# CrystalAnalyst/Lsm

Hardware: AMD Instinct MI355X
Metric: GiB/s device-resident SSTable block encode+decode, 4 KiB blocks, 1/2/4/8 GPU (higher is better)
Workload: dtype u8; 1 GPU; U: 1048576 blocks/GPU x block_size 4096, decode + re-encode (16-B uniform keys, 100-B values); blocks_per_gpu=1048576, entries_per_gpu=32474205, encoded_bytes_per_gpu=4226189427, decoded_bytes_per_gpu=4286595060, block_size=4096, segments_per_gpu=2045, parallelism=block-sharded x1 (no data-path collective), encode_output=segments packed (lsmblk_encode_batch), rccl_world=1

## Files before the change

### lsm_amd/csrc/lsmblk_dev.hpp

```cpp
#pragma once

#include <hip/hip_runtime.h>
#include <hip/hip_ext.h>

#include <cstdint>
#include <cstdlib>
#include <cstring>
#include <mutex>
#include <new>
#include <type_traits>
#include <vector>

#include "lsmblk.h"
#include "lsmblk_keys.hpp"

namespace {

constexpr uint32_t kSpinLimit = 1u << 22;

constexpr bool kDiag = LSMBLK_DIAG_BUILD != 0;
__device__ __forceinline__ uint32_t diag_mask(uint32_t skip) { return kDiag ? skip : 0u; }

__device__ __forceinline__ uint32_t lane_id() { return threadIdx.x & 63u; }
__device__ __forceinline__ uint32_t uni(uint32_t x) { return __builtin_amdgcn_readfirstlane(x); }
// ... 695 lines not shown
      cap = bytes = 0;
    }
    const hipError_t e = status ? hipExtMallocWithFlags(&mem, nb, kStatusFlags) : hipMallocAsync(&mem, nb, st);
    if (e != hipSuccess) {
      mem = nullptr;
      return LSMBLK_E_NOMEM;
    }
    if (fresh) *fresh = true;
    if (hipMemsetAsync(mem, 0, nb, st) != hipSuccess) return LSMBLK_E_HIP;
    cap = nc;
    bytes = nb;
    return LSMBLK_OK;
  }
  bool zero(hipStream_t st) const { return !bytes || hipMemsetAsync(mem, 0, bytes, st) == hipSuccess; }
  void release() {
    if (!mem) return;
    if (status) (void)hipFree(mem);
    else (void)hipFreeAsync(mem, nullptr);
    mem = nullptr;
    cap = bytes = 0;
  }
};
template <typename T>
struct DevBuf : DevBufBase {
  using DevBufBase::DevBufBase;
  T* get() const { return static_cast<T*>(mem); }
  operator T*() const { return get(); }
  int grow(hipStream_t st, uint64_t need, uint64_t per, bool* fresh = nullptr) {
    return grow_bytes(st, need, per * sizeof(T), fresh);
  }
};

struct lsmblk_ctx {
  int device = 0;
  std::mutex mu;
  DevBufBase* bufs = nullptr;
  uint32_t* counters = nullptr;
  DevBuf<uint32_t> dec_agg{bufs, false};
  void* crc_tabs = nullptr;
  DevBuf<uint64_t> tile_sum{bufs, false};
  DevBuf<uint64_t> tile_pre{bufs, false};
  DevBuf<uint64_t> seg_agg{bufs, true};
  DevBuf<uint64_t> seg_inc{bufs, true};
  DevBuf<uint32_t> rec_first{bufs, false};
  DevBuf<uint32_t> blk_first{bufs, false};
  DevBuf<uint32_t> ent{bufs, false};
  DevBuf<uint32_t> big_list{bufs, false};
  DevBuf<uint32_t> blk_sz{bufs, false};
  DevBuf<uint64_t> frec{bufs, true};
  DevBuf<uint64_t> fdone{bufs, true};
  DevBuf<uint32_t> fwnb{bufs, false};
  DevBuf<uint8_t> fbig{bufs, false};
  bool fuse_on = false;
  bool plan_pipe = false;
  uint32_t emit_mode = 0;
  uint32_t emit_grid = 0;
  DevBuf<uint64_t> lag_gran{bufs, true};
  uint64_t lag_blk_cap = 0;
  uint32_t rot_poison = 0;
  uint32_t emit_poison = 0;
  bool dec_two_pass = false;
  uint32_t dec_lag = kDecLagDefault;
  uint64_t dec_lag_bytes = kDecLagBytesDefault;
  uint64_t* dbg = nullptr;
  bool dbg_on = false;
  uint32_t epoch = 0;
  uint32_t poll = 0;
  uint32_t skip = 0;
  bool timing = false;
  struct KLog {
    const char* name;
    int slot;
    hipEvent_t e0, e1;
  };
  std::vector<KLog> klog;
  uint64_t klog_n = 0;
  uint64_t klog_total = 0;
  uint64_t dec_log0 = 0, dec_log1 = 0, enc_log0 = 0, enc_log1 = 0;
  DevBuf<uint32_t> meta_rec{bufs, false};
  DevBuf<uint64_t> meta_pos{bufs, false};
  DevBuf<uint64_t> meta_tile{bufs, false};
  DevBuf<uint32_t> meta_crc{bufs, false};
  uint64_t* meta_cstats = nullptr;
  DevBuf<uint32_t> filt_keep{bufs, false};
  DevBuf<uint64_t> filt_tile{bufs, false};
  DevBuf<uint8_t> cws{bufs, false};
  DevBuf<uint32_t> vcrc{bufs, false};
  hipStream_t aux = nullptr;
  hipEvent_t fork_ev = nullptr, join_ev = nullptr;
  DevBuf<uint8_t> sws{bufs, false};
  uint32_t scan_units = kScanUnitsDefault;
  DevBuf<uint8_t> rws{bufs, false};
  uint64_t shard_n = 0, shard_m = 0, shard_target = 0;
  uint32_t shard_block_size = 0, shard_flags = 0, shard_sst_cap = 0;
  bool shard_ready = false;
};

inline thread_local lsmblk_ctx* tl_launch_ctx = nullptr;
constexpr uint32_t kKLogCap = 16384;

namespace {
struct DeviceGuard {
  int prev = -1;
  bool ok = false;
  lsmblk_ctx* prev_ctx = nullptr;
  explicit DeviceGuard(int dev, lsmblk_ctx* c = nullptr) {
    if (hipGetDevice(&prev) != hipSuccess) prev = -1;
// ... 135 lines not shown
```

### lsm_amd/csrc/lsmblk_gpu.hip

```cpp
#include "lsmblk_dev.hpp"

namespace {


struct DecodeArgs {
  const uint8_t* blocks;
  const uint64_t* blk_off;
  uint64_t nblk;
  uint8_t* keys;
  uint32_t* key_off;
  uint8_t* vals;
  uint32_t* val_off;
  uint64_t* ts;
  uint64_t entry_cap, key_cap, val_cap;
  uint64_t* stats;
  const uint32_t* agg;
  const uint64_t* tile_pre;
  uint32_t tail;
  uint64_t* blk_ent;
  uint32_t skip;
  uint64_t* bagg;
  uint64_t* bbase;
  uint64_t* tagg;
  uint64_t* tinc;
// ... 1182 lines not shown
#pragma unroll
            for (uint32_t d = 0; d < 4; ++d) t[d] = uint32_t(__builtin_ctzg(P[d] ^ Q[d], 32)) >> 3;
            const uint32_t z16 = t[0] < 4 ? t[0] : t[1] < 4 ? 4 + t[1] : t[2] < 4 ? 8 + t[2] : 12 + t[3];
            const uint32_t zd = z16 >> 2;
            if (z16 < m) {
              lcp = z16;
              w0 = zd == 0 ? P[0] : zd == 1 ? P[1] : zd == 2 ? P[2] : P[3];
              w1 = zd == 0 ? Q[0] : zd == 1 ? Q[1] : zd == 2 ? Q[2] : Q[3];
            }
            done = z16 < m || m <= 16;
            if (!done) {
              for (uint32_t d = 4; 4 * d < m; ++d) {
                const uint32_t y0 = K.dw(pp[i] + 4 * d), y1 = K.dw(kp[i] + 4 * d);
                if (y0 != y1) {
                  const uint32_t z = 4 * d + (__builtin_ctz(y0 ^ y1) >> 3);
                  if (z < m) {
                    lcp = z;
                    w0 = y0;
                    w1 = y1;
                  }
                  break;
                }
              }
            }
          } else {
            const KeyDiff kd = key_diff(K, pp[i], pl, kp[i], kl);
            lcp = kd.lcp, w0 = kd.w0, w1 = kd.w1;
          }
          const uint32_t sh = 8 * (lcp & 3);
          const bool sorted = lcp == m ? pl <= kl : ((w0 >> sh) & 0xFF) < ((w1 >> sh) & 0xFF);
          al = (lcp < kAlcpLcp ? lcp : kAlcpLcp) | (sorted ? 0u : kAlcpUnsorted);
        }
        CR[x] = inv ? kl : kl + (v1[i] - v0[i]);
        CA[x] = al;
      }
    }
    __builtin_amdgcn_fence(__ATOMIC_RELEASE, "workgroup");
    if (l == 0) __hip_atomic_store(prod, cend - s0, __ATOMIC_RELAXED, __HIP_MEMORY_SCOPE_WORKGROUP);
  }
  if (tr && l == 0) {
    tr[5] = __builtin_amdgcn_s_memrealtime();
    tr[6] = waited;
  }
}

struct WalkRing {
  const uint32_t* CR;
  const uint32_t* CA;
  uint32_t* cons;
  const uint32_t* prod;
  uint32_t S0;
  uint32_t known = 0;
  bool stalled = false;
};

template <class Sink>
__device__ __forceinline__ void walk_segment(const PlanArgs& a, const ArenaKeys& K, WalkRing& R, uint32_t s0, uint32_t s1,
                                             uint32_t& err, uint32_t& nb, uint64_t& bytes, Sink&& sink, uint64_t* tr,
                                             uint64_t& waited, uint64_t& windows) {
  const uint32_t l = lane_id();
  auto need = [&](uint32_t j0, uint32_t wend) {
    __hip_atomic_store(R.cons, j0 - R.S0, __ATOMIC_RELAXED, __HIP_MEMORY_SCOPE_WORKGROUP);
    if (tr) ++windows;
    if (wend - R.S0 > R.known && !R.stalled) {
      const uint64_t w0 = tr ? __builtin_amdgcn_s_memrealtime() : 0;
      uint32_t spins = 0;
      while ((R.known = __hip_atomic_load(R.prod, __ATOMIC_RELAXED, __HIP_MEMORY_SCOPE_WORKGROUP)) < wend - R.S0) {
        if (++spins > kSpinMax) {
          err |= LSMBLK_ERR_TIMEOUT;
          R.stalled = true;
          break;
        }
        __builtin_amdgcn_s_sleep(1);
      }
      if (tr) waited += __builtin_amdgcn_s_memrealtime() - w0;
      __builtin_amdgcn_fence(__ATOMIC_ACQUIRE, "workgroup");
    }
  };
  const uint32_t* const CR = R.CR;
  const uint32_t* const CA = R.CA;
  const uint32_t S0 = R.S0;
  nb = 0;
  bytes = 0;
  const uint64_t bs = a.block_size;
  const bool narrow = bs < (1ull << 30);
  for (uint32_t s = s0; s < s1;) {
    uint64_t carry = 2;
    uint32_t pmin = kAlcpLcp;
    bool direct = false;
    uint32_t sp = 0, sl = 0;
    uint32_t j0 = s;
    const uint32_t aend = s1 - s < 64 ? s1 : s + 64;
    need(s, aend);
    if (!(diag_mask(a.skip) & (1u << 17))) {
      const bool valid = s + l < s1;
      uint32_t r = 0, al = kAlcpLcp;
      if (valid) {
        const uint32_t x = (s + l - S0) & (kRing - 1);
        r = CR[x];
        if (l) al = CA[x];
      }
      if (narrow && __ballot((al & kAlcpUnsorted) || (valid && r >= (1u << 25) - 16)) == 0) {
        const uint32_t mn = wave_incl_min31(al);
        const uint32_t g32 = valid ? r + 16 - (l ? mn : 0u) : 0u;
        const uint32_t i32 = wave_incl_scan32(g32);
        const uint32_t b32 = 2 + i32 - g32;
        const uint64_t m = __ballot(l && (!valid || b32 + r + 14 > uint32_t(bs)));
        if (m) {
          const uint32_t f = uint32_t(__builtin_ctzll(m));
          const uint32_t size = uint32_t(__builtin_amdgcn_readlane(b32, f));
          sink(s, s + f, size, nb, bytes);
          ++nb;
          bytes += size;
          s += f;
          continue;
// ... 179 lines not shown
      if (kl == 0) err |= LSMBLK_ERR_EMPTY_KEY;
      uint32_t al = 0;
      if (e != s0) {
        const uint32_t pl = kp - pp, m = pl < kl ? pl : kl;
        uint32_t lcp = m, w0 = 0, w1 = 0;
        if (K.lead + kp + 16 <= klim && K.lead + pp + 16 <= klim) {
          const uint32_t Pw[4] = {xp[i].x, xp[i].y, xp[i].z, xp[i].w}, Qw[4] = {xk[i].x, xk[i].y, xk[i].z, xk[i].w};
          uint32_t t[4];
#pragma unroll
          for (uint32_t d = 0; d < 4; ++d) t[d] = uint32_t(__builtin_ctzg(Pw[d] ^ Qw[d], 32)) >> 3;
          const uint32_t z16 = t[0] < 4 ? t[0] : t[1] < 4 ? 4 + t[1] : t[2] < 4 ? 8 + t[2] : 12 + t[3];
          const uint32_t zd = z16 >> 2;
          if (z16 < m) {
            lcp = z16;
            w0 = zd == 0 ? Pw[0] : zd == 1 ? Pw[1] : zd == 2 ? Pw[2] : Pw[3];
            w1 = zd == 0 ? Qw[0] : zd == 1 ? Qw[1] : zd == 2 ? Qw[2] : Qw[3];
          }
          if (!(z16 < m || m <= 16)) {
            for (uint32_t d = 4; 4 * d < m; ++d) {
              const uint32_t y0 = K.dw(pp + 4 * d), y1 = K.dw(kp + 4 * d);
              if (y0 != y1) {
                const uint32_t z = 4 * d + (__builtin_ctz(y0 ^ y1) >> 3);
                if (z < m) {
                  lcp = z;
                  w0 = y0;
                  w1 = y1;
                }
                break;
              }
            }
          }
        } else {
          const KeyDiff kd = key_diff(K, pp, pl, kp, kl);
          lcp = kd.lcp, w0 = kd.w0, w1 = kd.w1;
        }
        const uint32_t sh = 8 * (lcp & 3);
        const bool sorted = lcp == m ? pl <= kl : ((w0 >> sh) & 0xFF) < ((w1 >> sh) & 0xFF);
        al = (lcp < kAlcpLcp ? lcp : kAlcpLcp) | (sorted ? 0u : kAlcpUnsorted);
      }
      CR[x] = inv ? kl : kl + (P.v1[i] - P.v0[i]);
      CA[x] = al;
    }
    __builtin_amdgcn_fence(__ATOMIC_RELEASE, "workgroup");
    if (l == 0) __hip_atomic_store(prod, cend - s0, __ATOMIC_RELAXED, __HIP_MEMORY_SCOPE_WORKGROUP);
    prod_offs_land(Pn);
    P = Pn;
  }
  if (tr && l == 0) {
    tr[5] = __builtin_amdgcn_s_memrealtime();
    tr[6] = waited;
  }
}

__global__ __launch_bounds__(kWalkThreads) __attribute__((amdgpu_waves_per_eu(4))) void plan_walk_kernel(PlanArgs a0) {
  const PlanArgs a = resolve(a0);
  static_assert(kRing >= 2 * kChunk && (kRing & (kRing - 1)) == 0, "plan ring size");
  __shared__ uint32_t crec[4][kRing], calcp[4][kRing];
  const uint32_t l = lane_id();
  __shared__ uint32_t hand_g[4], hand_prod[4], hand_cons[4];
  const uint32_t wv = wave_id(), ww = wv & 3;
  if (wv < 4) {
    const uint32_t t = take_ticket(a.ticket);
    if (l == 0) {
      hand_g[wv] = t;
      hand_prod[wv] = 0;
      hand_cons[wv] = 0;
    }
  }
  __syncthreads();
  const uint32_t g = uni(hand_g[ww]);
  uint32_t* CR = crec[ww];
  uint32_t* CA = calcp[ww];
  if (g >= a.nseg) return;
  uint32_t err = 0;
  uint32_t s0 = uni(a.seg_start[g]), s1 = uni(a.seg_start[g + 1]);
  if ((!a.span && g == 0 && s0 != 0) || (!a.span && g == a.nseg - 1 && uint64_t(s1) != a.n) || s0 > s1 ||
      uint64_t(s1) > a.n) {
    err |= LSMBLK_ERR_SEGMENTS;
    s1 = s0 = (s0 > a.n ? uint32_t(a.n) : s0);
    if (s1 < s0) s1 = s0;
  }
  const ArenaKeys K = plan_keys(a);
  uint64_t* const tr = kDiag && a.dbg && g < kDbgTiles ? a.dbg + 16 + 8 * uint64_t(g) : nullptr;
  if (wv >= 4) {
    if (a.pipe_helper) plan_produce_pipe(a, K, s0, s1, CR, CA, &hand_prod[ww], &hand_cons[ww], err, tr);
    else plan_produce(a, K, s0, s1, CR, CA, &hand_prod[ww], &hand_cons[ww], err, tr);
    const uint32_t werr = (__ballot(err & LSMBLK_ERR_EMPTY_KEY) ? LSMBLK_ERR_EMPTY_KEY : 0u) |
                          (__ballot(err & LSMBLK_ERR_MALFORMED) ? LSMBLK_ERR_MALFORMED : 0u) |
                          (__ballot(err & LSMBLK_ERR_TIMEOUT) ? LSMBLK_ERR_TIMEOUT : 0u);
    raise_err(a.stats, werr);
    return;
  }
  uint64_t waited = 0, windows = 0;
  if (tr && l == 0) tr[0] = __builtin_amdgcn_s_memrealtime();
  WalkRing R{CR, CA, &hand_cons[ww], &hand_prod[ww], s0};
  uint32_t nb = 0;
  uint64_t bytes = 0;
  walk_segment(a, K, R, s0, s1, err, nb, bytes,
               [&](uint32_t first, uint32_t, uint32_t size, uint32_t i, uint64_t) {
                 if (l == 0) {
                   a.rec_first[s0 + i] = first;
                   a.sz[s0 + i] = size;
                 }
               },
               tr, waited, windows);
  if (tr && l == 0) {
    tr[1] = __builtin_amdgcn_s_memrealtime();
    tr[2] = waited;
    tr[3] = windows;
    tr[7] = nb | (uint64_t(__builtin_amdgcn_s_getreg(0xF804)) << 32) | (uint64_t(__builtin_amdgcn_s_getreg(0x1814) & 0xF) << 56);
  }
  bytes += uint64_t(a.frame) * nb;
  __builtin_amdgcn_fence(__ATOMIC_RELEASE, "agent");
  asm volatile("s_waitcnt vmcnt(0)" ::: "memory");
  __builtin_amdgcn_fence(__ATOMIC_ACQUIRE, "agent");
  uint64_t agg[2] = {nb, bytes};
  uint64_t excl[2] = {0, 0};
  if (g == 0) {
    publish<2>(a.inc, g, agg, a.tag, 2, a.poll);
  } else {
    publish<2>(a.agg, g, agg, a.tag, 1, a.poll);
    if (!lookback<2>(a.agg, a.inc, g, a.tag, a.poll, excl)) err |= LSMBLK_ERR_TIMEOUT;
    const uint64_t inc[2] = {excl[0] + agg[0], excl[1] + agg[1]};
    publish<2>(a.inc, g, inc, a.tag, 2, a.poll);
  }
  uint64_t O0 = excl[1];
  if (a.seg_out) O0 = (err & LSMBLK_ERR_SEGMENTS) ? 0ull : seg_slot(a.key_off, a.val_off, 0u, s0, a.frame);
  const uint64_t B0 = excl[0];
  if (a.seg_out && l == 0) {
    a.seg_out[2ull * g] = O0;
    a.seg_out[2ull * g + 1] = bytes;
  }
  uint64_t oc = O0;
  for (uint32_t c = 0; c < nb; c += 64) {
    const uint32_t i = c + l;
    uint32_t sz = 0, first = 0;
    if (i < nb) {
      first = a.rec_first[s0 + i];
      sz = a.sz[s0 + i];
    }
    const uint64_t ext = i < nb ? uint64_t(sz) + a.frame : 0ull;
    const uint64_t incl = wave_incl_scan<uint64_t>(ext);
    if (i < nb) {
      const uint64_t bi = B0 + i;
      a.blk_first[bi] = first;
      if (a.blk_sz) a.blk_sz[bi] = sz;
      if (bi < a.blk_cap) a.blk_off[bi] = oc + incl - ext;
    }
    oc += __shfl(incl, 63, 64);
  }
  if (g == a.nseg - 1 && l == 0) {
    const uint64_t Bt = B0 + nb, Ot = O0 + bytes;
    a.blk_first[Bt] = a.span ? s1 : uint32_t(a.n);
    if (Bt < a.blk_cap) a.blk_off[Bt] = Ot;
    a.stats[0] = Bt;
    a.stats[1] = excl[1] + bytes;
    if (Bt + 1 > a.blk_cap || Ot > a.out_cap) err |= LSMBLK_ERR_CAPACITY;
  }
// ... 648 lines not shown
    y = ny;
    fp = nfp;
    fl = nfl;
  }
  raise_err(a.stats, err);
}

__global__ __launch_bounds__(256) void emit_poison_kernel(uint32_t* blk_first, const uint64_t* stats) {
  if (stats[3] & kPlanFatal) return;
  const uint64_t nblk = stats[0], b = 1 + 5 * (uint64_t(blockIdx.x) * 256 + threadIdx.x);
  if (b < nblk) blk_first[b] = blk_first[b + 1] + 1;
}

struct FuseArgs {
  PlanArgs p;
  EmitArgs e;
  uint64_t* rec;
  uint64_t* wdone;
  uint32_t* wnb;
  uint64_t* seg_out;
  uint8_t* bigr;
  uint32_t nwalk;
  uint32_t spw;
  uint32_t walk_wgs;
  uint32_t per_walker;
};
static_assert(4 * kRing * 4 + 16 <= sizeof(EmitLds) * kEmitWaves, "two walkers' rings fit emit's LDS");

__device__ __forceinline__ uint32_t walker_first_seg(const FuseArgs& f, uint32_t w) {
  return uint32_t(min(uint64_t(w) * f.spw, uint64_t(f.p.nseg)));
}
__device__ __forceinline__ uint32_t walker_rbase(const FuseArgs& f, uint32_t w) {
  return f.p.seg_start[walker_first_seg(f, w)] - f.p.seg_start[0] + w;
}

__device__ void fuse_walk(const FuseArgs& f, uint32_t* ring) {
  const PlanArgs& a = f.p;
  const uint32_t l = lane_id(), wv = wave_id(), ww = wv & 1;
  uint32_t* CR = ring + ww * kRing;
  uint32_t* CA = ring + (2 + ww) * kRing;
  uint32_t* prod = ring + 4 * kRing + ww;
  uint32_t* cons = ring + 4 * kRing + 2 + ww;
  const uint32_t w = 2 * blockIdx.x + ww;
  const uint32_t g0 = walker_first_seg(f, w), g1 = uint32_t(min(uint64_t(g0) + f.spw, uint64_t(a.nseg)));
  uint32_t err = 0;
  bool ok = uni(a.seg_start[0]) == 0;
  for (uint32_t g = g0; g < g1; ++g) {
    const uint32_t s0 = uni(a.seg_start[g]), s1 = uni(a.seg_start[g + 1]);
    if ((g == 0 && s0 != 0) || (g == a.nseg - 1 && uint64_t(s1) != a.n) || s0 > s1 || uint64_t(s1) > a.n) ok = false;
  }
  const uint32_t S0 = ok ? uni(a.seg_start[g0]) : 0u, S1 = ok ? uni(a.seg_start[g1]) : 0u;
  const ArenaKeys K = plan_keys(a);
  if (wv >= 2) {
    plan_produce_pipe(a, K, S0, S1, CR, CA, prod, cons, err);
    const uint32_t werr = (__ballot(err & LSMBLK_ERR_EMPTY_KEY) ? LSMBLK_ERR_EMPTY_KEY : 0u) |
                          (__ballot(err & LSMBLK_ERR_MALFORMED) ? LSMBLK_ERR_MALFORMED : 0u) |
                          (__ballot(err & LSMBLK_ERR_TIMEOUT) ? LSMBLK_ERR_TIMEOUT : 0u);
    raise_err(a.stats, werr);
    return;
  }
  if (!ok) err |= LSMBLK_ERR_SEGMENTS;
  WalkRing R{CR, CA, cons, prod, S0};
  const uint32_t rb = walker_rbase(f, w);
  const uint64_t tagb = uint64_t(a.tag) << 2;
  uint32_t nbw = 0;
  uint64_t waited = 0, windows = 0;
  uint64_t* const tr = kDiag && a.dbg && w < kDbgTiles ? a.dbg + 16 + 8 * uint64_t(w) : nullptr;
  if (tr && l == 0) tr[0] = __builtin_amdgcn_s_memrealtime();
  for (uint32_t g = g0; ok && g < g1; ++g) {
    const uint32_t s0 = uni(a.seg_start[g]), s1 = uni(a.seg_start[g + 1]);
    const uint64_t slot = seg_slot(a.key_off, a.val_off, 0u, s0);
    uint32_t nb = 0;
    uint64_t bytes = 0;
    walk_segment(a, K, R, s0, s1, err, nb, bytes,
                 [&](uint32_t first, uint32_t end, uint32_t size, uint32_t i, uint64_t before) {
                   const uint64_t v = l == 0 ? first : (l == 1 ? end : (l == 2 ? slot + before : size));
                   if (l < 4) gstore(f.rec + 4ull * (rb + nbw + i) + l, (v << 16) | tagb | 1, a.poll);
                 },
                 tr, waited, windows);
    if (l == 0) {
      f.seg_out[2ull * g] = slot;
      f.seg_out[2ull * g + 1] = bytes;
    }
    nbw += nb;
  }
  if (l == 0) {
    f.wnb[w] = nbw;
    gstore(f.wdone + w, (uint64_t(nbw) << 16) | tagb | 2, a.poll);
    if (tr) {
      tr[1] = __builtin_amdgcn_s_memrealtime();
      tr[2] = waited;
      tr[3] = windows;
      tr[4] = nbw;
    }
  }
  raise_err(a.stats, err);
}

__device__ void fuse_emit(const FuseArgs& f, EmitLds& L) {
  const EmitArgs& a = f.e;
  const uint32_t l = lane_id();
  const uint32_t eidx = (blockIdx.x - f.walk_wgs) * kEmitWaves + wave_id();
  const uint32_t w = eidx % f.nwalk, r = f.per_walker;
  uint32_t it = eidx / f.nwalk;
  if (it >= r) return;
  const uint32_t g0 = walker_first_seg(f, w), g1 = uint32_t(min(uint64_t(g0) + f.spw, uint64_t(f.p.nseg)));
  const uint32_t S0 = uni(f.p.seg_start[g0]), S1 = uni(f.p.seg_start[g1]);
// ... 1012 lines not shown
  }
  ++c->epoch;
  return LSMBLK_OK;
}

bool aligned16(const void* p) { return (reinterpret_cast<uintptr_t>(p) & 15) == 0; }

int ensure_cstats(lsmblk_ctx* c) {
  if (c->meta_cstats || hipMalloc(reinterpret_cast<void**>(&c->meta_cstats), LSMBLK_STATS_WORDS * 8) == hipSuccess)
    return LSMBLK_OK;
  c->meta_cstats = nullptr;
  return LSMBLK_E_NOMEM;
}

int filt_prepare(lsmblk_ctx* c, const lsmblk_kv_stream* in, const lsmblk_kv_stream* out, uint64_t* stats,
                 hipStream_t st, FiltArgs& a) {
  const uint64_t ntiles = (in->n + kFiltTile - 1) / kFiltTile;
  int rc;
  if ((rc = c->filt_keep.grow(st, in->n + 1, 1)) || (rc = c->filt_tile.grow(st, ntiles + 1, 6))) return rc;
  memset(&a, 0, sizeof(a));
  a.keys = in->keys;
  a.key_off = in->key_off;
  a.vals = in->vals;
  a.val_off = in->val_off;
  a.ts = in->ts;
  a.n = in->n;
  a.okeys = out->keys;
  a.okey_off = out->key_off;
  a.ovals = out->vals;
  a.oval_off = out->val_off;
  a.ots = out->ts;
  a.entry_cap = out->entry_cap;
  a.key_cap = out->key_cap;
  a.val_cap = out->val_cap;
  a.keep = c->filt_keep;
  a.tile_sum = c->filt_tile;
  a.tile_pre = c->filt_tile + 3 * c->filt_tile.cap;
  a.stats = stats;
  return LSMBLK_OK;
}

}

extern "C" {

int lsmblk_ctx_create(int device, lsmblk_ctx** out) {
  if (!out) return LSMBLK_E_INVAL;
  int ndev = 0;
  if (hipGetDeviceCount(&ndev) != hipSuccess || device < 0 || device >= ndev) return LSMBLK_E_HIP;
  auto* c = new (std::nothrow) lsmblk_ctx();
  if (!c) return LSMBLK_E_NOMEM;
  c->device = device;
  if (const char* e = getenv("LSMBLK_POLL_MODE")) c->poll = uint32_t(atoi(e));
  if (const char* e = getenv("LSMBLK_PLAN_PIPE")) c->plan_pipe = atoi(e) != 0;
  if (const char* e = getenv("LSMBLK_EMIT_MODE")) {
    const unsigned long v = strtoul(e, nullptr, 0);
    if ((v & 0xFF) <= 2 && v <= 0xFFFFFFFFul) c->emit_mode = uint32_t(v & 0xFF), c->emit_grid = uint32_t(v >> 8);
  }
  DeviceGuard dg(device);
  if (!dg.ok || hipMalloc(&c->counters, 2048) != hipSuccess) {
    delete c;
    return LSMBLK_E_HIP;
  }
  *out = c;
  return LSMBLK_OK;
}

void lsmblk_ctx_destroy(lsmblk_ctx* c) {
  if (!c) return;
  DeviceGuard dg(c->device, c);
  (void)hipDeviceSynchronize();
  if (c->aux) (void)hipStreamDestroy(c->aux);
  if (c->fork_ev) (void)hipEventDestroy(c->fork_ev);
  if (c->join_ev) (void)hipEventDestroy(c->join_ev);
  (void)hipFree(c->counters);
  (void)hipFree(c->crc_tabs);
  (void)hipFree(c->meta_cstats);
  for (DevBufBase* b = c->bufs; b; b = b->next) b->release();
  (void)hipStreamSynchronize(nullptr);
  (void)hipFree(c->dbg);
  for (auto& e : c->klog) {
    if (e.e0) (void)hipEventDestroy(e.e0);
    if (e.e1) (void)hipEventDestroy(e.e1);
  }
  delete c;
}

int lsmblk_debug_set(lsmblk_ctx* c, int key, uint32_t value) {
  if (!c) return LSMBLK_E_INVAL;
  std::lock_guard<std::mutex> g(c->mu);
  if (key == LSMBLK_DEBUG_POLL_MODE && value <= 2) {
    c->poll = value;
  } else if (key == LSMBLK_DEBUG_DECODE_SKIP && kDiag) {
    c->skip = value;
  } else if (key == LSMBLK_DEBUG_TWO_PASS_DECODE) {
    c->dec_two_pass = value != 0;
  } else if (key == LSMBLK_DEBUG_COUNTERS && kDiag) {
    if (value && !c->dbg) {
      DeviceGuard dg(c->device, c);
      if (!dg.ok || hipMalloc(reinterpret_cast<void**>(&c->dbg), kDbgWords * 8) != hipSuccess) {
        c->dbg = nullptr;
        return LSMBLK_E_NOMEM;
      }
    }
    c->dbg_on = value != 0;
  } else if (key == LSMBLK_DEBUG_ROT_POISON && kDiag) {
    c->rot_poison = value;
  } else if (key == LSMBLK_DEBUG_EMIT_POISON && kDiag) {
    c->emit_poison = value;
  } else if (key == LSMBLK_DEBUG_DECODE_LAG_BYTES) {
    c->dec_lag_bytes = value;
  } else if (key == LSMBLK_DEBUG_DECODE_LAG && value == 0) {
    c->dec_lag = kDecLagDefault;
    c->dec_lag_bytes = kDecLagBytesDefault;
  } else if (key == LSMBLK_DEBUG_DECODE_LAG && value >= 2 * kTile && value <= (1u << 24)) {
    c->dec_lag = value;
    c->dec_lag_bytes = 0;
  } else if (key == LSMBLK_DEBUG_ENCODE_FUSED) {
    c->fuse_on = value != 0;
  } else if (key == LSMBLK_DEBUG_PLAN_PIPE) {
    c->plan_pipe = value != 0;
  } else if (key == LSMBLK_DEBUG_EMIT_MODE && (value & 0xFF) <= 2) {
    c->emit_mode = value & 0xFF;
    c->emit_grid = value >> 8;
  } else if (key == LSMBLK_DEBUG_SCAN_UNITS && value <= (1u << 24)) {
    c->scan_units = value ? value : kScanUnitsDefault;
  } else if (key == LSMBLK_DEBUG_KERNEL_TIMING) {
    if (value && !c->timing) c->klog_n = 0;
    c->timing = value != 0;
  } else {
    return LSMBLK_E_INVAL;
  }
  return LSMBLK_OK;
}

int lsmblk_debug_counters(lsmblk_ctx* c, uint64_t* out, uint32_t n) {
  if (!c || !out || n > kDbgWords) return LSMBLK_E_INVAL;
  std::lock_guard<std::mutex> g(c->mu);
  for (uint32_t i = 0; i < n; ++i) out[i] = 0;
  if (!c->dbg) return LSMBLK_OK;
  DeviceGuard dg(c->device, c);
  if (!dg.ok || hipDeviceSynchronize() != hipSuccess) return LSMBLK_E_HIP;
  return hipMemcpy(out, c->dbg, n * 8, hipMemcpyDeviceToHost) == hipSuccess ? LSMBLK_OK : LSMBLK_E_HIP;
}

int lsmblk_ctx_kernel_times(lsmblk_ctx* c, float* ms) {
  if (!c || !ms) return LSMBLK_E_INVAL;
  std::lock_guard<std::mutex> g(c->mu);
  for (int i = 0; i < LSMBLK_KERNELS; ++i) ms[i] = -1.f;
  if (c->klog.empty()) return LSMBLK_OK;
  DeviceGuard dg(c->device);
  if (!dg.ok) return LSMBLK_E_HIP;
  auto add = [&](uint64_t i0, uint64_t i1) -> int {
    if (c->klog_total - i0 > kKLogCap) return LSMBLK_OK;
    for (uint64_t i = i0; i < i1; ++i) {
      const lsmblk_ctx::KLog& e = c->klog[i % kKLogCap];
      if (e.slot < 0 || e.slot >= LSMBLK_KERNELS) continue;
      float t = 0.f;
      if (hipEventSynchronize(e.e1) != hipSuccess || hipEventElapsedTime(&t, e.e0, e.e1) != hipSuccess)
        return LSMBLK_E_HIP;
      ms[e.slot] = (ms[e.slot] < 0.f ? 0.f : ms[e.slot]) + t;
    }
    return LSMBLK_OK;
  };
  const int rc = add(c->dec_log0, c->dec_log1);
  return rc ? rc : add(c->enc_log0, c->enc_log1);
}

int lsmblk_ctx_kernel_log(lsmblk_ctx* c, lsmblk_kernel_stat* out, uint32_t cap, uint32_t* n) {
  if (!c || !n || (cap && !out)) return LSMBLK_E_INVAL;
  std::lock_guard<std::mutex> g(c->mu);
  *n = 0;
  const uint64_t cnt = c->klog_n;
  c->klog_n = 0;
// ... 175 lines not shown
  if (framed && (q.span || q.dn || q.dnseg)) return LSMBLK_E_INVAL;
  int rc = reserve_locked(c, 0, in->n, q.nseg, st);
  if (rc) return rc;
  if (hipMemsetAsync(q.stats, 0, LSMBLK_STATS_WORDS * 8, st) != hipSuccess) return LSMBLK_E_HIP;
  if (q.nseg == 0) {
    if (in->n != 0) return LSMBLK_E_INVAL;
    if (q.blk_cap >= 1 && hipMemsetAsync(q.blk_off, 0, 8, st) != hipSuccess) return LSMBLK_E_HIP;
    return LSMBLK_OK;
  }
  const int cus = cu_count(c);
  const bool fused = slots && !framed && q.block_size <= 4096 && c->fuse_on;
  uint32_t walk_wgs = 0, nwalk = 0;
  if (fused) {
    walk_wgs = uint32_t(std::min<uint64_t>(uint64_t(cus), (uint64_t(q.nseg) + 1) / 2));
    walk_wgs += walk_wgs & 1;
    nwalk = 2 * walk_wgs;
    const uint64_t recs = in->n + nwalk + 1;
    bool fresh = false;
    rc = c->frec.grow(st, recs, 4, &fresh);
    if (!rc) rc = c->fdone.grow(st, nwalk, 1, &fresh);
    if (fresh) c->epoch = 0;
    if (rc || (rc = c->fwnb.grow(st, nwalk, 1)) || (rc = c->fbig.grow(st, recs, 1))) return rc;
  }
  if (framed && (rc = ensure_crc_tabs(c, st))) return rc;
  if ((rc = next_epoch(c, st))) return rc;
  if (hipMemsetAsync(c->counters, 0, 2048, st) != hipSuccess) return LSMBLK_E_HIP;
  PlanArgs p;
  p.keys = in->keys;
  p.key_off = in->key_off;
  p.val_off = in->val_off;
  p.n = in->n;
  p.seg_start = q.seg_start;
  p.nseg = q.nseg;
  p.block_size = q.block_size;
  p.sz = c->ent;
  p.rec_first = c->rec_first;
  p.blk_first = c->blk_first;
  p.blk_off = q.blk_off;
  p.blk_cap = q.blk_cap;
  p.out_cap = q.out_cap;
  p.stats = q.stats;
  p.ticket = c->counters + 256;
  p.agg = c->seg_agg;
  p.inc = c->seg_inc;
  p.tag = c->epoch;
  p.poll = c->poll;
  p.dn = q.dn;
  p.dnseg = q.dnseg;
  p.span = q.span ? 1u : 0u;
  p.skip = c->skip;
  p.dbg = c->dbg_on ? c->dbg : nullptr;
  p.seg_out = slots ? q.seg_out : nullptr;
  p.blk_sz = slots || framed ? c->blk_sz : nullptr;
  p.pipe_helper = c->plan_pipe ? 1u : 0u;
  p.frame = framed ? 4u : 0u;
  EmitArgs e;
  e.keys = in->keys;
  e.key_off = in->key_off;
  e.vals = in->vals;
  e.val_off = in->val_off;
  e.ts = in->ts;
  e.blk_first = c->blk_first;
  e.blk_off = q.blk_off;
  e.out = q.out;
  e.out_cap = q.out_cap;
  e.blk_cap = q.blk_cap;
  e.n = in->n;
  e.stats = q.stats;
  e.big_flag = reinterpret_cast<uint8_t*>(c->big_list.get());
  e.blk_sz = slots || framed ? c->blk_sz : nullptr;
  e.skip = c->skip;
  e.dn = q.dn;
  if (fused) {
    if (p.dbg && hipMemsetAsync(p.dbg, 0, kDbgWords * 8, st) != hipSuccess) return LSMBLK_E_HIP;
    FuseArgs f;
    f.p = p;
    f.e = e;
    f.rec = c->frec;
    f.wdone = c->fdone;
    f.wnb = c->fwnb;
    f.seg_out = q.seg_out;
    f.bigr = c->fbig;
    f.nwalk = nwalk;
    f.spw = uint32_t((uint64_t(q.nseg) + nwalk - 1) / nwalk);
    f.walk_wgs = walk_wgs;
    f.per_walker = std::max<uint32_t>(1u, uint32_t(3ull * kEmitWaves * uint64_t(cus) / nwalk));
    const uint32_t emit_wgs = f.per_walker * nwalk / kEmitWaves;
    LSM_LAUNCH_SLOT(4, encode_fused_kernel, dim3(walk_wgs + emit_wgs), dim3(256), 0, st, f);
    LSM_LAUNCH(slot_tables_kernel, dim3(nwalk), dim3(256), 0, st, f, c->blk_first.get(), c->blk_sz.get(),
               reinterpret_cast<uint8_t*>(c->big_list.get()), q.blk_off, q.blk_cap, q.out_cap);
  } else {
    if (p.dbg && hipMemsetAsync(p.dbg, 0, kDbgWords * 8, st) != hipSuccess) return LSMBLK_E_HIP;
    LSM_LAUNCH_SLOT(3, plan_walk_kernel, dim3((q.nseg + 3) / 4), dim3(kWalkThreads), 0, st, p);
    if (c->skip & (3u << 16)) {
      return launch_rc();
    }
    if (kDiag && c->emit_poison)
      LSM_LAUNCH(emit_poison_kernel, dim3(uint32_t(in->n / (5 * 256) + 1)), dim3(256), 0, st, c->blk_first.get(), q.stats);
    const uint64_t nblk_max = q.blk_cap < in->n + 1 ? q.blk_cap : in->n + 1;
    if (nblk_max && hipMemsetAsync(c->big_list, 0, nblk_max, st) != hipSuccess) return LSMBLK_E_HIP;
    if (launch_rc()) return LSMBLK_E_HIP;
    if ((c->emit_mode ? c->emit_mode : kEmitModeDefault) == 2) {
      const uint64_t clamp = c->emit_grid ? c->emit_grid : kEmitGridMax;
      const uint32_t grid = uint32_t(std::max<uint64_t>(1, std::min(nblk_max, clamp)));
      LSM_LAUNCH_SLOT(4, emit_block_kernel, dim3(grid), dim3(64), 0, st, e);
    } else {
      LSM_LAUNCH_SLOT(4, emit_kernel, dim3(resident_wgs(cus, emit_kernel, 256, 3)), dim3(256), 0, st, e);
// ... 239 lines not shown
```

Measured before the change: 1032 GiB/s.

## Add run-batched prefetching plan producer and batch walker output stores

Adds a new plan producer in which each lane handles four consecutive entries. It loads key offsets, keys and value offsets with wide buffer loads issued one batch ahead, uses DPP to get neighbour keys, and writes 16-byte vectors into the LDS ring. This producer becomes the default (plan_pipe=0), and the old pipe and plain producers are now selected by values 1 and 2. The walker publishes its consumer position to the producer less often, and rec_first/sz are gathered across lanes and written 64 at a time instead of one lane per record. The aim is to hide global-load latency and cut store and LDS traffic in the plan stage, at the cost of more registers and more complex ring synchronisation.

Result: no change. 1041 GiB/s, median of 6 (+0.9%).

```diff
diff --git a/lsm_amd/csrc/lsmblk_dev.hpp b/lsm_amd/csrc/lsmblk_dev.hpp
--- a/lsm_amd/csrc/lsmblk_dev.hpp
+++ b/lsm_amd/csrc/lsmblk_dev.hpp
@@ -771,7 +771,7 @@
   DevBuf<uint32_t> fwnb{bufs, false};
   DevBuf<uint8_t> fbig{bufs, false};
   bool fuse_on = false;
-  bool plan_pipe = false;
+  uint32_t plan_pipe = 0;
   uint32_t emit_mode = 0;
   uint32_t emit_grid = 0;
   DevBuf<uint64_t> lag_gran{bufs, true};
diff --git a/lsm_amd/csrc/lsmblk_gpu.hip b/lsm_amd/csrc/lsmblk_gpu.hip
--- a/lsm_amd/csrc/lsmblk_gpu.hip
+++ b/lsm_amd/csrc/lsmblk_gpu.hip
@@ -1258,6 +1258,7 @@
   uint32_t S0;
   uint32_t known = 0;
   bool stalled = false;
+  uint32_t pub = 0;
 };
 
 template <class Sink>
@@ -1266,7 +1267,10 @@
                                              uint64_t& waited, uint64_t& windows) {
   const uint32_t l = lane_id();
   auto need = [&](uint32_t j0, uint32_t wend) {
-    __hip_atomic_store(R.cons, j0 - R.S0, __ATOMIC_RELAXED, __HIP_MEMORY_SCOPE_WORKGROUP);
+    if (j0 - R.S0 - R.pub >= kChunk || (wend - R.S0 > R.known && !R.stalled)) {
+      __hip_atomic_store(R.cons, j0 - R.S0, __ATOMIC_RELAXED, __HIP_MEMORY_SCOPE_WORKGROUP);
+      R.pub = j0 - R.S0;
+    }
     if (tr) ++windows;
     if (wend - R.S0 > R.known && !R.stalled) {
       const uint64_t w0 = tr ? __builtin_amdgcn_s_memrealtime() : 0;
@@ -1552,10 +1556,211 @@
   }
 }
 
+__device__ __forceinline__ uint32_t pair_alcp(const ArenaKeys& K, uint32_t klim, uint32_t pp, uint32_t pl, uint32_t kp,
+                                              uint32_t kl, const u32x4& xp, const u32x4& xk) {
+  const uint32_t m = pl < kl ? pl : kl;
+  uint32_t lcp = m, w0 = 0, w1 = 0;
+  if (K.lead + kp + 16 <= klim && K.lead + pp + 16 <= klim) {
+    const uint32_t Pw[4] = {xp.x, xp.y, xp.z, xp.w}, Qw[4] = {xk.x, xk.y, xk.z, xk.w};
+    uint32_t t[4];
+#pragma unroll
+    for (uint32_t d = 0; d < 4; ++d) t[d] = uint32_t(__builtin_ctzg(Pw[d] ^ Qw[d], 32)) >> 3;
+    const uint32_t z16 = t[0] < 4 ? t[0] : t[1] < 4 ? 4 + t[1] : t[2] < 4 ? 8 + t[2] : 12 + t[3];
+    const uint32_t zd = z16 >> 2;
+    if (z16 < m) {
+      lcp = z16;
+      w0 = zd == 0 ? Pw[0] : zd == 1 ? Pw[1] : zd == 2 ? Pw[2] : Pw[3];
+      w1 = zd == 0 ? Qw[0] : zd == 1 ? Qw[1] : zd == 2 ? Qw[2] : Qw[3];
+    }
+    if (!(z16 < m || m <= 16)) {
+      for (uint32_t d = 4; 4 * d < m; ++d) {
+        const uint32_t y0 = K.dw(pp + 4 * d), y1 = K.dw(kp + 4 * d);
+        if (y0 != y1) {
+          const uint32_t z = 4 * d + (__builtin_ctz(y0 ^ y1) >> 3);
+          if (z < m) {
+            lcp = z;
+            w0 = y0;
+            w1 = y1;
+          }
+          break;
+        }
+      }
+    }
+  } else {
+    const KeyDiff kd = key_diff(K, pp, pl, kp, kl);
+    lcp = kd.lcp, w0 = kd.w0, w1 = kd.w1;
+  }
+  const uint32_t sh = 8 * (lcp & 3);
+  const bool sorted = lcp == m ? pl <= kl : ((w0 >> sh) & 0xFF) < ((w1 >> sh) & 0xFF);
+  return (lcp < kAlcpLcp ? lcp : kAlcpLcp) | (sorted ? 0u : kAlcpUnsorted);
+}
+
+constexpr uint32_t kRunLen = 4;
+constexpr uint32_t kRunE = 64 * kRunLen;
+constexpr uint32_t kRunAhead = 1;
+static_assert(kRing % kRunE == 0 && kRing >= 2 * kRunE && kRunLen == 4, "ring holds whole batches of 16-byte groups");
+struct RunKeys {
+  u32x4 x[kRunLen];
+  u32x4 vo;
+  uint32_t vn;
+};
+__device__ __forceinline__ uint32_t run_index(uint32_t c, uint32_t s1) {
+  const uint32_t e = c + kRunLen * lane_id();
+  return 4 * (e < s1 ? e : s1);
+}
+__device__ __forceinline__ void run_offs_issue(const rsrc_t& RKO, uint32_t c, uint32_t s1, u32x4& ko) {
+  asm volatile("buffer_load_dwordx4 %0, %1, %2, 0 offen" : "=&v"(ko) : "v"(run_index(c, s1)), "s"(RKO));
+}
+__device__ __forceinline__ void run_keys_issue(const rsrc_t& RK, uint32_t lead, const rsrc_t& RVO, uint32_t c, uint32_t s1,
+                                               const u32x4& ko, RunKeys& X) {
+  const uint32_t o0 = lead + ko.x, o1 = lead + ko.y, o2 = lead + ko.z, o3 = lead + ko.w;
+  asm volatile(
+      "buffer_load_dwordx4 %0, %6, %11, 0 offen\n\t"
+      "buffer_load_dwordx4 %1, %7, %11, 0 offen\n\t"
+      "buffer_load_dwordx4 %2, %8, %11, 0 offen\n\t"
+      "buffer_load_dwordx4 %3, %9, %11, 0 offen\n\t"
+      "buffer_load_dwordx4 %4, %10, %12, 0 offen\n\t"
+      "buffer_load_dword %5, %10, %12, 0 offen offset:16"
+      : "=&v"(X.x[0]), "=&v"(X.x[1]), "=&v"(X.x[2]), "=&v"(X.x[3]), "=&v"(X.vo), "=&v"(X.vn)
+      : "v"(o0), "v"(o1), "v"(o2), "v"(o3), "v"(run_index(c, s1)), "s"(RK), "s"(RVO));
+}
+__device__ __forceinline__ void run_move(u32x4& d, const u32x4& s) {
+  asm volatile(
+      "v_mov_b32 %0, %4\n\t"
+      "v_mov_b32 %1, %5\n\t"
+      "v_mov_b32 %2, %6\n\t"
+      "v_mov_b32 %3, %7"
+      : "=&v"(d.x), "=&v"(d.y), "=&v"(d.z), "=&v"(d.w)
+      : "v"(s.x), "v"(s.y), "v"(s.z), "v"(s.w));
+}
+__device__ void plan_produce_run(const PlanArgs& a, const ArenaKeys& K, uint32_t s0, uint32_t s1, uint32_t* CR,
+                                 uint32_t* CA, uint32_t* prod, const uint32_t* cons, uint32_t& err,
+                                 uint64_t* tr = nullptr) {
+  const uint32_t l = lane_id();
+  const uint32_t klim = K.lead + uni(a.key_off[a.n]);
+  uint64_t waited = 0;
+  if (tr && l == 0) tr[4] = __builtin_amdgcn_s_memrealtime();
+  if (s0 >= s1) return;
+  const bool noloads = diag_mask(a.skip) & (1u << 18), nokeys = noloads || (diag_mask(a.skip) & (1u << 16));
+  const uint32_t nb4 = uint32_t(min(uint64_t(a.n + 1) * 4, uint64_t(0xFFFFFFF0u)));
+  const rsrc_t RKO = make_rsrc_exact(const_cast<uint32_t*>(a.key_off), noloads ? 0u : nb4);
+  const rsrc_t RVO = make_rsrc_exact(const_cast<uint32_t*>(a.val_off), noloads ? 0u : nb4);
+  const rsrc_t RK = nokeys ? make_rsrc_exact(nullptr, 0u) : K.r;
+  auto next = [&](uint32_t c) { return s1 - c > kRunE ? c + kRunE : s1; };
+  u32x4 Kc, Kn, Kf;
+  RunKeys X, Xf;
+  auto land = [&]() {
+    asm volatile("s_waitcnt vmcnt(0)" ::: "memory");
+    asm volatile("" : "+v"(Kf), "+v"(Xf.x[0]), "+v"(Xf.x[1]), "+v"(Xf.x[2]), "+v"(Xf.x[3]), "+v"(Xf.vo), "+v"(Xf.vn));
+  };
+  asm volatile("s_nop 4" ::: "memory");
+  run_offs_issue(RKO, s0, s1, Kf);
+  asm volatile("s_waitcnt vmcnt(0)" ::: "memory");
+  asm volatile("" : "+v"(Kf));
+  run_move(Kn, Kf);
+  run_keys_issue(RK, K.lead, RVO, s0, s1, Kn, Xf);
+  run_offs_issue(RKO, next(s0), s1, Kf);
+  uint32_t cpp = 0, ckey[4] = {0, 0, 0, 0};
+  for (uint32_t c = s0; c < s1; c += kRunE) {
+    const uint32_t cend = s1 - c < kRunE ? s1 : c + kRunE;
+    if (c - s0 + kRunE > kRing && !(err & LSMBLK_ERR_TIMEOUT)) {
+      const uint32_t need = c - s0 + kRunE - kRing;
+      uint32_t spins = 0;
+      const uint64_t w0 = tr ? __builtin_amdgcn_s_memrealtime() : 0;
+      while (__hip_atomic_load(cons, __ATOMIC_RELAXED, __HIP_MEMORY_SCOPE_WORKGROUP) < need) {
+        if (++spins > kSpinMax) {
+          err |= LSMBLK_ERR_TIMEOUT;
+          break;
+        }
+        __builtin_amdgcn_s_sleep(1);
+      }
+      if (tr) waited += __builtin_amdgcn_s_memrealtime() - w0;
+      __builtin_amdgcn_fence(__ATOMIC_ACQUIRE, "workgroup");
+    }
+    land();
+    Kc = Kn;
+    run_move(Kn, Kf);
+    run_move(X.x[0], Xf.x[0]);
+    run_move(X.x[1], Xf.x[1]);
+    run_move(X.x[2], Xf.x[2]);
+    run_move(X.x[3], Xf.x[3]);
+    run_move(X.vo, Xf.vo);
+    asm volatile("v_mov_b32 %0, %1" : "=&v"(X.vn) : "v"(Xf.vn));
+    const uint32_t c1 = next(c);
+    if (kRunAhead) {
+      run_keys_issue(RK, K.lead, RVO, c1, s1, Kn, Xf);
+      run_offs_issue(RKO, next(c1), s1, Kf);
+    }
+    const uint32_t e0 = c + kRunLen * l;
+    uint32_t pp = LSM_DPP(Kc.w, 0x138, 0xF);
+    uint32_t kn = LSM_DPP(Kc.x, 0x130, 0xF);
+    u32x4 xp;
+    xp.x = LSM_DPP(X.x[3].x, 0x138, 0xF);
+    xp.y = LSM_DPP(X.x[3].y, 0x138, 0xF);
+    xp.z = LSM_DPP(X.x[3].z, 0x138, 0xF);
+    xp.w = LSM_DPP(X.x[3].w, 0x138, 0xF);
+    if (l == 0) {
+      pp = cpp;
+      xp = u32x4{ckey[0], ckey[1], ckey[2], ckey[3]};
+    }
+    if (l == 63) kn = __builtin_amdgcn_readlane(Kn.x, 0);
+    cpp = __builtin_amdgcn_readlane(Kc.w, 63);
+    ckey[0] = __builtin_amdgcn_readlane(X.x[3].x, 63);
+    ckey[1] = __builtin_amdgcn_readlane(X.x[3].y, 63);
+    ckey[2] = __builtin_amdgcn_readlane(X.x[3].z, 63);
+    ckey[3] = __builtin_amdgcn_readlane(X.x[3].w, 63);
+    const uint32_t ko[6] = {pp, Kc.x, Kc.y, Kc.z, Kc.w, kn};
+    const uint32_t vo[5] = {X.vo.x, X.vo.y, X.vo.z, X.vo.w, X.vn};
+    uint32_t rec[kRunLen], alc[kRunLen];
+#pragma unroll
+    for (uint32_t i = 0; i < kRunLen; ++i) {
+      const uint32_t e = e0 + i;
+      rec[i] = alc[i] = 0;
+      if (e >= cend) continue;
+      if (noloads) {
+        rec[i] = 120;
+        alc[i] = e != s0 ? 8u : 0u;
+        continue;
+      }
+      const uint32_t kp = ko[i + 1];
+      const bool inv = ko[i + 2] < kp || vo[i + 1] < vo[i];
+      if (inv) err |= LSMBLK_ERR_MALFORMED;
+      const uint32_t kl = inv ? 1u : ko[i + 2] - kp;
+      if (kl == 0) err |= LSMBLK_ERR_EMPTY_KEY;
+      if (e != s0 && !nokeys) alc[i] = pair_alcp(K, klim, ko[i], kp - ko[i], kp, kl, i ? X.x[i ? i - 1 : 0] : xp, X.x[i]);
+      rec[i] = inv ? kl : kl + (vo[i + 1] - vo[i]);
+    }
+    const uint32_t x = (e0 - s0) & (kRing - 1);
+    if (e0 + kRunLen <= cend) {
+      *reinterpret_cast<u32x4*>(CR + x) = u32x4{rec[0], rec[1], rec[2], rec[3]};
+      *reinterpret_cast<u32x4*>(CA + x) = u32x4{alc[0], alc[1], alc[2], alc[3]};
+    } else {
+#pragma unroll
+      for (uint32_t i = 0; i < kRunLen; ++i) {
+        if (e0 + i < cend) {
+          CR[x + i] = rec[i];
+          CA[x + i] = alc[i];
+        }
+      }
+    }
+    __builtin_amdgcn_fence(__ATOMIC_RELEASE, "workgroup");
+    if (l == 0) __hip_atomic_store(prod, cend - s0, __ATOMIC_RELAXED, __HIP_MEMORY_SCOPE_WORKGROUP);
+    if (!kRunAhead) {
+      run_keys_issue(RK, K.lead, RVO, c1, s1, Kn, Xf);
+      run_offs_issue(RKO, next(c1), s1, Kf);
+    }
+  }
+  asm volatile("s_waitcnt vmcnt(0)" ::: "memory");
+  if (tr && l == 0) {
+    tr[5] = __builtin_amdgcn_s_memrealtime();
+    tr[6] = waited;
+  }
+}
+
 __global__ __launch_bounds__(kWalkThreads) __attribute__((amdgpu_waves_per_eu(4))) void plan_walk_kernel(PlanArgs a0) {
   const PlanArgs a = resolve(a0);
   static_assert(kRing >= 2 * kChunk && (kRing & (kRing - 1)) == 0, "plan ring size");
-  __shared__ uint32_t crec[4][kRing], calcp[4][kRing];
+  __shared__ alignas(16) uint32_t crec[4][kRing], calcp[4][kRing];
   const uint32_t l = lane_id();
   __shared__ uint32_t hand_g[4], hand_prod[4], hand_cons[4];
   const uint32_t wv = wave_id(), ww = wv & 3;
@@ -1583,7 +1788,8 @@
   const ArenaKeys K = plan_keys(a);
   uint64_t* const tr = kDiag && a.dbg && g < kDbgTiles ? a.dbg + 16 + 8 * uint64_t(g) : nullptr;
   if (wv >= 4) {
-    if (a.pipe_helper) plan_produce_pipe(a, K, s0, s1, CR, CA, &hand_prod[ww], &hand_cons[ww], err, tr);
+    if (a.pipe_helper == 0) plan_produce_run(a, K, s0, s1, CR, CA, &hand_prod[ww], &hand_cons[ww], err, tr);
+    else if (a.pipe_helper == 1) plan_produce_pipe(a, K, s0, s1, CR, CA, &hand_prod[ww], &hand_cons[ww], err, tr);
     else plan_produce(a, K, s0, s1, CR, CA, &hand_prod[ww], &hand_cons[ww], err, tr);
     const uint32_t werr = (__ballot(err & LSMBLK_ERR_EMPTY_KEY) ? LSMBLK_ERR_EMPTY_KEY : 0u) |
                           (__ballot(err & LSMBLK_ERR_MALFORMED) ? LSMBLK_ERR_MALFORMED : 0u) |
@@ -1596,14 +1802,22 @@
   WalkRing R{CR, CA, &hand_cons[ww], &hand_prod[ww], s0};
   uint32_t nb = 0;
   uint64_t bytes = 0;
+  uint32_t rfirst = 0, rsize = 0;
   walk_segment(a, K, R, s0, s1, err, nb, bytes,
                [&](uint32_t first, uint32_t, uint32_t size, uint32_t i, uint64_t) {
-                 if (l == 0) {
-                   a.rec_first[s0 + i] = first;
-                   a.sz[s0 + i] = size;
+                 const bool mine = l == (i & 63);
+                 rfirst = mine ? first : rfirst;
+                 rsize = mine ? size : rsize;
+                 if ((i & 63) == 63) {
+                   a.rec_first[s0 + i - 63 + l] = rfirst;
+                   a.sz[s0 + i - 63 + l] = rsize;
                  }
                },
                tr, waited, windows);
+  if (l < (nb & 63)) {
+    a.rec_first[s0 + (nb & ~63u) + l] = rfirst;
+    a.sz[s0 + (nb & ~63u) + l] = rsize;
+  }
   if (tr && l == 0) {
     tr[1] = __builtin_amdgcn_s_memrealtime();
     tr[2] = waited;
@@ -2358,7 +2572,8 @@
   const uint32_t S0 = ok ? uni(a.seg_start[g0]) : 0u, S1 = ok ? uni(a.seg_start[g1]) : 0u;
   const ArenaKeys K = plan_keys(a);
   if (wv >= 2) {
-    plan_produce_pipe(a, K, S0, S1, CR, CA, prod, cons, err);
+    if (a.pipe_helper == 0) plan_produce_run(a, K, S0, S1, CR, CA, prod, cons, err);
+    else plan_produce_pipe(a, K, S0, S1, CR, CA, prod, cons, err);
     const uint32_t werr = (__ballot(err & LSMBLK_ERR_EMPTY_KEY) ? LSMBLK_ERR_EMPTY_KEY : 0u) |
                           (__ballot(err & LSMBLK_ERR_MALFORMED) ? LSMBLK_ERR_MALFORMED : 0u) |
                           (__ballot(err & LSMBLK_ERR_TIMEOUT) ? LSMBLK_ERR_TIMEOUT : 0u);
@@ -3477,7 +3692,7 @@
   if (!c) return LSMBLK_E_NOMEM;
   c->device = device;
   if (const char* e = getenv("LSMBLK_POLL_MODE")) c->poll = uint32_t(atoi(e));
-  if (const char* e = getenv("LSMBLK_PLAN_PIPE")) c->plan_pipe = atoi(e) != 0;
+  if (const char* e = getenv("LSMBLK_PLAN_PIPE")) c->plan_pipe = uint32_t(atoi(e)) <= 2 ? uint32_t(atoi(e)) : 0u;
   if (const char* e = getenv("LSMBLK_EMIT_MODE")) {
     const unsigned long v = strtoul(e, nullptr, 0);
     if ((v & 0xFF) <= 2 && v <= 0xFFFFFFFFul) c->emit_mode = uint32_t(v & 0xFF), c->emit_grid = uint32_t(v >> 8);
@@ -3543,8 +3758,8 @@
     c->dec_lag_bytes = 0;
   } else if (key == LSMBLK_DEBUG_ENCODE_FUSED) {
     c->fuse_on = value != 0;
-  } else if (key == LSMBLK_DEBUG_PLAN_PIPE) {
-    c->plan_pipe = value != 0;
+  } else if (key == LSMBLK_DEBUG_PLAN_PIPE && value <= 2) {
+    c->plan_pipe = value;
   } else if (key == LSMBLK_DEBUG_EMIT_MODE && (value & 0xFF) <= 2) {
     c->emit_mode = value & 0xFF;
     c->emit_grid = value >> 8;
@@ -3826,7 +4041,7 @@
   p.dbg = c->dbg_on ? c->dbg : nullptr;
   p.seg_out = slots ? q.seg_out : nullptr;
   p.blk_sz = slots || framed ? c->blk_sz : nullptr;
-  p.pipe_helper = c->plan_pipe ? 1u : 0u;
+  p.pipe_helper = c->plan_pipe;
   p.frame = framed ? 4u : 0u;
   EmitArgs e;
   e.keys = in->keys;
```
